# emiliofidalgo/liodom

Hardware: AMD Instinct MI355X
Metric: scans/sec (64×1800 cloud, prev_frames=20) at 1 GPU; pose RMSE vs CPU ref (higher is better)
Workload: dtype f64

## Files before the change

liodom_amd/csrc/kernels_lm.h:

```cpp
constexpr int kLmWaves = kLmThreads / 64;
__host__ __device__ __forceinline__ size_t lm_lds_bytes(int edge_cap) {
  return (size_t)((edge_cap + 3) & ~3) * sizeof(int);
}


__device__ int lm_compact_bits(const DevView& v, int s, int outer_it, int E, int* idx ) {
  const int lane = threadIdx.x & 63;
  const int Q = v.knn_queries;
  const int nb = (E + Q - 1) / Q;
  const int nwords = (nb + 3) >> 2;
  const unsigned int* mw = reinterpret_cast<const unsigned int*>(v.corr_mask + ((size_t)s * 2 + outer_it) * v.mask_stride);
  int run = 0;
  for (int w0 = 0; w0 < nwords; w0 += 64) {
    const int w = w0 + lane;
    unsigned int word = (w < nwords) ? mw[w] : 0u;
    const int pop = __popc(word);
    const int incl = wave_incl_scan_i32(pop);
    int o = run + incl - pop;
    while (word) {
      const int b = __ffs(word) - 1;
      word &= word - 1u;
      const int bit = w * 32 + b;
      idx[o++] = (bit >> 3) * Q + (bit & 7);
    }
// ... 112 lines not shown
__device__ __forceinline__ void finalize_scan(const DevView& v, int s, StreamState& st, int* sh_cnt, int eb, bool clear_hash, int ctl, int chain,
                              const double* T, int raw, bool publish_pose, const double* prev, int fc_old, int pred_copies = 3, unsigned int verdict = 1u,
                              const liodom_lm_trace_t* trace1 = nullptr) {
  __shared__ double sh_pred[19];
  const int P = v.prev_frames;
  const int tid = threadIdx.x;
  const int fc_new = fc_old + 1;
  const int nf = fc_new < P ? fc_new : P;
  const int new_slot = fc_old % P;
  int* wn = v.win_n + (size_t)s * P;
  int* wb = v.win_base + (size_t)s * (P + 1);
  int* ws = v.win_slot + (size_t)s * P;
  if (publish_pose && v.early_rebuild && tid < 50) publish_final_pose(v, s, T, raw, (unsigned int)fc_old + 1u, tid % 25, tid / 25);
  const int n_edges = st.n_edges_buf[eb];
  const int nup = st.n_used_tab[0];
  for (int j = tid; j < nf; j += blockDim.x) {
    const int sl = (fc_new - nf + j) % P;
    sh_cnt[j] = (sl == new_slot) ? n_edges : wn[sl];
    ws[j] = sl;
  }
  if (tid == 64) {
    double fin[12], q[4];
    for (int i = 0; i < 12; i++) fin[i] = T[i];
    quat_from_pose(fin, v.rotation_mode, q);
    const int k = st.scan_counter;
    st.info.scan_index = k;
    st.info.status = st.status;
    if (trace1) st.info.lm[1] = *trace1;
    if (k < v.pose_log_cap) {
      double* pl = v.pose_log + ((size_t)s * v.pose_log_cap + k) * 7;
      pl[0] = q[0]; pl[1] = q[1]; pl[2] = q[2]; pl[3] = q[3];
      pl[4] = fin[3]; pl[5] = fin[7]; pl[6] = fin[11];
      v.info_log[(size_t)s * v.pose_log_cap + k] = st.info;
    }
    st.scan_counter = k + 1;
    if (v.host_out) {
      HostOut* ho = v.host_out + (size_t)s * 2 + (k & 1);
      ho->pose[0] = q[0]; ho->pose[1] = q[1]; ho->pose[2] = q[2]; ho->pose[3] = q[3];
      ho->pose[4] = fin[3]; ho->pose[5] = fin[7]; ho->pose[6] = fin[11];
      ho->info = st.info;
      ho->pad = (int)verdict;
      __hip_atomic_store(&ho->seq, k + 1, __ATOMIC_RELEASE, __HIP_MEMORY_SCOPE_SYSTEM);
    }
    st.info.matches[0] = 0; st.info.matches[1] = 0;
  }
  if (tid == ctl) {
    double po[12];
    for (int i = 0; i < 12; i++) po[i] = prev ? prev[i] : st.prev_odom[i];
    predict_next(T, po, v.rotation_mode, sh_pred);
  }
  __syncthreads();
  if (v.pred_xch) { pred_publish(v, s, sh_pred, (unsigned int)fc_new, tid, (int)blockDim.x, pred_copies); pred_verdict_publish(v, s, (unsigned int)fc_new, verdict, tid); }
  if (tid == ctl) {
    for (int i = 0; i < 12; i++) { const double f = T[i]; st.final_odom[i] = f; st.prev_odom[i] = f; st.odom[i] = sh_pred[i]; }
    for (int i = 0; i < 4; i++) st.param_q[i] = sh_pred[12 + i];
    st.param_t[0] = sh_pred[16]; st.param_t[1] = sh_pred[17]; st.param_t[2] = sh_pred[18];
    wn[new_slot] = n_edges;
    st.frame_count = fc_new;
    st.n_frames = nf;
    int acc = 0;
    for (int j = 0; j < nf; j++) { const int c = sh_cnt[j]; sh_cnt[j] = acc; acc += c; }
    sh_cnt[nf] = acc;
    st.n_map = acc;
    if (!v.early_rebuild) st.n_used_tab[0] = 0;
    else { st.n_search = acc; st.n_filt = 0; }
    if (!chain) st.cursor = 0;
  }
  __syncthreads();
  for (int j = tid; j <= nf; j += blockDim.x) wb[j] = sh_cnt[j];
  if (clear_hash && !v.early_rebuild) hash_clear_used(v, s, nup, tid, (int)blockDim.x);
}

__device__ __forceinline__ unsigned int xcc_id() { return (unsigned int)__builtin_amdgcn_s_getreg(20 | (0 << 6) | (3 << 11)) & 0xFu; }
__device__ bool lm_exchange(const DevView& v, int s, int g, int G, unsigned int epoch,
                            double x, double* acc_total, unsigned int* status, bool local, int lane) {
  typedef __attribute__((address_space(1))) unsigned long long gu64;
  unsigned long long* base = v.lm_xch + ((size_t)s * 2 + (epoch & 1u)) * kLmGroupsMax * 64;
  INJECT_DELAY(16);
  if (lane <= 2 * kAccN) {
    unsigned long long half;
    if (lane < 2 * kAccN) {
      const unsigned long long bits = (unsigned long long)__double_as_longlong(x);
      half = (lane & 1) ? (bits >> 32) : (bits & 0xFFFFFFFFull);
    } else {
      half = xcc_id();
    }
    const unsigned long long word = ((unsigned long long)epoch << 32) | half;
    if (local) __hip_atomic_store((gu64*)(base + g * 64 + lane), word, __ATOMIC_RELAXED, __HIP_MEMORY_SCOPE_WORKGROUP);
    else __hip_atomic_store((gu64*)(base + g * 64 + lane), word, __ATOMIC_RELAXED, __HIP_MEMORY_SCOPE_AGENT);
  }
  double tot = 0.0;
  unsigned int spins = 0;
  unsigned long long t0w = 0;
  bool same = true;
  while (true) {
    bool ok = true;
    tot = 0.0;
    same = true;
    if (lane <= kAccN) {
      unsigned long long lo[kLmGroupsMax], hi[kLmGroupsMax];
      const int i0 = lane < kAccN ? 2 * lane : 2 * kAccN, i1 = lane < kAccN ? 2 * lane + 1 : 2 * kAccN;
#pragma unroll
      for (int gg = 0; gg < kLmGroupsMax; gg++) {
        const int gq = gg < G ? gg : 0;
        lo[gg] = __hip_atomic_load((gu64*)(base + gq * 64 + i0), __ATOMIC_RELAXED, __HIP_MEMORY_SCOPE_AGENT);
        hi[gg] = __hip_atomic_load((gu64*)(base + gq * 64 + i1), __ATOMIC_RELAXED, __HIP_MEMORY_SCOPE_AGENT);
      }
#pragma unroll
      for (int gg = 0; gg < kLmGroupsMax; gg++) {
        if (gg < G) {
          ok = ok && ((unsigned int)(lo[gg] >> 32) == epoch) && ((unsigned int)(hi[gg] >> 32) == epoch);
          tot += __longlong_as_double((long long)((hi[gg] << 32) | (lo[gg] & 0xFFFFFFFFull)));
          same = same && ((unsigned int)lo[gg] == (unsigned int)lo[0]);
        }
      }
    }
    if (__all(ok)) break;
    if (++spins > 4000000u || __any(wait_expired(spins, t0w))) { if (lane == 0) atomicOr(status, LIODOM_STATUS_LM_SYNC_TIMEOUT); same = false; break; }
    __builtin_amdgcn_s_sleep(1);
  }
  if (lane < kAccN) acc_total[lane] = tot;
  return __builtin_amdgcn_readlane((int)same, kAccN) != 0;
}

__device__ __forceinline__ void publish_final_pose(const DevView& v, int s, const double* T, int raw, unsigned int tag, int lane , int copy) {
  typedef __attribute__((address_space(1))) unsigned long long gu64;
  unsigned long long* base = v.pose_xch + (size_t)s * 64 + copy * 32;
  INJECT_DELAY(15);
  unsigned int word = (unsigned int)raw;
  if (lane < 24) {
    const unsigned long long bits = (unsigned long long)__double_as_longlong(T[lane >> 1]);
    word = (lane & 1) ? (unsigned int)(bits >> 32) : (unsigned int)bits;
  }
  __hip_atomic_store((gu64*)(base + lane), ((unsigned long long)tag << 32) | word, __ATOMIC_RELAXED, __HIP_MEMORY_SCOPE_AGENT);
}

__global__ void k_imu_override(DevView v, int s0, int count) {
  const int i = blockIdx.x * blockDim.x + threadIdx.x;
  if (i >= count) return;
  StreamState& st = v.state[s0 + i];
  if (!st.initialized) return;
  double odom[12], out[12], l2b[12], q[4];
#pragma unroll
  for (int k = 0; k < 12; k++) { odom[k] = st.odom[k]; l2b[k] = v.laser_to_base[k]; }
#pragma unroll
  for (int k = 0; k < 4; k++) q[k] = v.imu_q[(size_t)(s0 + i) * 4 + k];
  imu_override(odom, q, l2b, v.rotation_mode, out);
#pragma unroll
  for (int k = 0; k < 12; k++) st.odom[k] = out[k];
  quat_from_pose(out, v.rotation_mode, st.param_q);
  st.param_t[0] = out[3]; st.param_t[1] = out[7]; st.param_t[2] = out[11];
}

__device__ __forceinline__ void pose_cov_store(const DevView& v, int s, const StreamState& st, const LmState& lm, const double* acc, int nblocks, int tid) {
  const int j = tid - 64;
  if (j < 0 || j >= 21) return;
  PoseCovRaw* r = v.cov_raw + s;
  bool applied = lm.termination == LM_TERM_FUNC_TOL && lm.apply_on_ftol != 0;
  for (int k = 0; k < 4; k++) applied = applied && lm.q[k] == lm.cand_q[k];
  for (int k = 0; k < 3; k++) applied = applied && lm.t[k] == lm.cand_t[k];
  r->H[j] = applied ? acc[7 + j] : lm.H[j];
  if (j == 0) {
    r->scan_index = st.info.scan_index; r->n_res = nblocks; r->termination = lm.termination; r->has_solve = 1;
    r->cost = lm.cost;
  }
}

__device__ __forceinline__ void rebuild_beside_solve(const DevView& v, int s, StreamState& st, int eb, int outer_it, int block, int nblocks, unsigned int seq, int* sbase, int* sslot);

template <int kOuterIt, bool kChainMode>
#ifndef LIODOM_LM_WAVES_PER_SIMD
#define LIODOM_LM_WAVES_PER_SIMD 1
#endif
__global__ __launch_bounds__(kLmThreads, LIODOM_LM_WAVES_PER_SIMD) void k_lm_solve(DevView v, int s0, int eb, unsigned int seq, unsigned int done_target) {
  constexpr int outer_it = kOuterIt;
  constexpr int chain = kChainMode ? 1 : 0;
  __shared__ double sh_pose2[2][12];
  __shared__ int sh_pi, sh_ci;
  __shared__ int sh_nmoved;
  __shared__ double sh_pred_s[20];
  __shared__ int sh_unapplied;
  __shared__ double sh_acc[kAccN];
  __shared__ LmState lm;
  __shared__ int sh_flag;
  __shared__ int sh_C;
  const int s = s0 + blockIdx.y;
#if defined(LIODOM_CHAIN_PRIO)
  if (v.n_streams <= 4) __builtin_amdgcn_s_setprio(LIODOM_CHAIN_PRIO);
#endif
  const int G = v.lm_groups, gstride = G > 1 ? 8 : 1, bxl = (int)blockIdx.x;
  const bool is_solver = bxl < G * gstride && (bxl % gstride) == 0;
  const int g = is_solver ? bxl / gstride : G + (bxl < G * gstride ? bxl - (bxl / gstride + 1) : bxl - G);
  StreamState& st = v.state[s];
  __shared__ int sh_cnt[kMaxFrames + 1];
  OV_STAMP(v, bxl == 0 && threadIdx.x == 0, outer_it == 0 ? 0 : 3);
  if (seq && outer_it == 0 && bxl == 0 && threadIdx.x == 0) {
    typedef __attribute__((address_space(1))) unsigned int gu32;
    __hip_atomic_store((gu32*)(v.ov_flags + s), seq, __ATOMIC_RELAXED, __HIP_MEMORY_SCOPE_AGENT);
  }
  if (g >= G) {
    if (!v.early_rebuild || chain) return;
    __shared__ int sh_slot[kMaxFrames];
    rebuild_beside_solve(v, s, st, eb, outer_it, g - G, (int)gridDim.x - G, seq, sh_cnt, sh_slot);
    return;
  }
  __shared__ double sh_wsum[kLmWaves][32];
  __shared__ double sh_red[16][32];
  __shared__ double sh_x0[8];
  __shared__ double sh_prev[12];
  __shared__ int sh_fc;
  if (threadIdx.x < 4) sh_x0[threadIdx.x] = st.param_q[threadIdx.x];
  else if (threadIdx.x < 7) sh_x0[threadIdx.x] = st.param_t[threadIdx.x - 4];
  else if (threadIdx.x >= 64 && threadIdx.x < 76) sh_prev[threadIdx.x - 64] = st.prev_odom[threadIdx.x - 64];
  else if (threadIdx.x == 76) sh_fc = st.frame_count;
  __shared__ int sh_spec_at;
  if (threadIdx.x == 77) sh_spec_at = st.spec_eval[outer_it];
  __shared__ int sh_redo;
  if (threadIdx.x == 78) sh_redo = st.spec_redo[outer_it == 0 ? 1 : 0];
  extern __shared__ __attribute__((aligned(16))) int sh_idx[];
  const int tid = threadIdx.x;
  const bool prep = tid < kLmCtl;
  bool dead = false;
  if (chain && outer_it == 0) dead = !chain_wait_count(v.knn_done0 + s, done_target, &st.status);
  if (chain && outer_it == 0 && sh_redo) __builtin_amdgcn_fence(__ATOMIC_ACQUIRE, "agent");
  int E_in;
  if (chain && outer_it == 0) {
    typedef __attribute__((address_space(1))) unsigned int gu32;
    E_in = (int)__hip_atomic_load((gu32*)(v.edge_cnt + eb * 32 + s), __ATOMIC_RELAXED, __HIP_MEMORY_SCOPE_AGENT);
  } else {
    E_in = st.n_edges_buf[eb];
  }
  if (outer_it == 0 && tid == 0 && g == 0) {
    st.info.n_edges = E_in;
    st.info.map_points = st.n_search;
    for (int k = 0; k < 2; k++) {
      st.info.lm[k].iterations = 0; st.info.lm[k].accepted = 0; st.info.lm[k].termination = LM_TERM_NO_RESIDUALS;
      st.info.lm[k].pad = 0; st.info.lm[k].initial_cost = 0.0; st.info.lm[k].final_cost = 0.0;
    }
  }
  if (!st.initialized) {
    if (outer_it == 1 && g == 0) {
      if (seq) ov_wait_knn_done(v, s, seq, &st.status);
      if (tid == 0) st.append_raw = 1;
      __shared__ double sh_T0[12];
      if (tid < 12) sh_T0[tid] = st.odom[tid];
      __syncthreads();
      finalize_scan(v, s, st, sh_cnt, eb, true, 0, 0, sh_T0, 1, true, sh_prev, sh_fc);
      if (tid == 0) st.initialized = 1;
      if (v.cov_raw && tid == 64) {
        PoseCovRaw* r = v.cov_raw + s;
        r->scan_index = st.info.scan_index; r->n_res = 0; r->termination = st.info.lm[1].termination; r->has_solve = 0; r->cost = st.info.lm[1].final_cost;
      }
    }
    return;
  }
  bool clr_pending = outer_it == 1 && g == 0 && prep && !v.early_rebuild;
  auto clear_hash_slots = [&]() {
    hash_clear_used(v, s, st.n_used_tab[0], tid, kLmCtl);
    clr_pending = false;
  };
  const bool dbgb = (s == 0) && (g == 0) && (tid == kLmCtl) && (outer_it == 1);
  const bool dbge = (s == 0) && (g == 0) && (tid == 0) && (outer_it == 1);
  DBG_STAMP(v, dbgb, 2, 0);
  const int E = E_in;
  int nblocks = st.info.matches[outer_it];
  __shared__ int sh_nmatch;
  __shared__ double sh_scale[8];
  const unsigned int epoch0 = ((unsigned int)(st.scan_counter + 1) << 6) | ((unsigned int)outer_it << 5);
  unsigned int n_eval = 0;
  bool xch_local = false;
  LmCache cache;
  int c_lo = 0, c_hi = 0;
  int dbg_it = 0;
  auto evaluate = [&](const double* pose) {
    lm_eval(v, s, outer_it, eb, c_lo, c_hi, sh_idx, pose, &sh_wsum[0][0], cache);
    if (tid >= kLmCtl) {
      const int lane = tid - kLmCtl;
      if (G > 1) {
        const double x = lm_wave_total(&sh_wsum[0][0], c_hi - c_lo, lane >> 1);
        DBG_STAMP(v, dbgb && dbg_it < 4, 2, 12 + dbg_it);
        xch_local = lm_exchange(v, s, g, G, epoch0 | ++n_eval, x, sh_acc, &st.status, xch_local, lane);
      } else {
        if (lane < kAccN) sh_acc[lane] = lm_wave_total(&sh_wsum[0][0], c_hi - c_lo, lane);
        ++n_eval;
      }
      asm volatile("s_waitcnt lgkmcnt(0)" ::: "memory");
      __builtin_amdgcn_wave_barrier();
    }
  };
  auto my_share = [&](int C) {
    const int chunk = (C + G - 1) / G;
    c_lo = g * chunk < C ? g * chunk : C;
    c_hi = (g + 1) * chunk < C ? (g + 1) * chunk : C;
  };
  if (seq && outer_it == 1) { if (chain) dead = !chain_wait_count(v.knn_done0 + 32 + s, done_target, &st.status) || dead; else ov_wait_knn_done(v, s, seq, &st.status); }
  if (seq && outer_it == 1) { __syncthreads(); if (sh_redo) __builtin_amdgcn_fence(__ATOMIC_ACQUIRE, "agent"); }
  OV_STAMP(v, g == 0 && tid == 0 && outer_it == 1, 4);
  OV_STAMP(v, g == 0 && tid == 0 && outer_it == 0, 18);
  if (v.knn_partials) {
    const int Q = v.knn_queries;
    const int nb = (E + Q - 1) / Q;
    const double* part = v.knn_part + ((size_t)s * 2 + outer_it) * v.knn_blocks * 32;
    constexpr int kRC = kLmThreads / 32;
    const int i = tid & 31, r0 = tid >> 5;
    double x0 = 0.0, x1 = 0.0;
    if (i <= kAccN) {
      const int nb_cap = v.knn_blocks;
      for (int rb = r0; rb < (dead ? 0 : (rb == r0 ? nb_cap : nb)); rb += 16 * kRC) {
        double xs[16];
#pragma unroll
        for (int u = 0; u < 16; u++) { const int r = rb + kRC * u; xs[u] = (r < nb_cap) ? part[(size_t)r * 32 + i] : 0.0; }
#pragma unroll
        for (int u = 0; u < 16; u++) { const int r = rb + kRC * u; if (r >= nb) xs[u] = 0.0; }
#pragma unroll
        for (int u = 0; u < 16; u += 2) { x0 += xs[u]; x1 += xs[u + 1]; }
      }
    }
    sh_red[r0][i] = x0 + x1;
    __syncthreads();
    if (tid <= kAccN) {
      double x = 0.0;
#pragma unroll
      for (int r = 0; r < kRC; r++) x += sh_red[r][tid];
      if (tid < kAccN) sh_acc[tid] = x;
      else { sh_nmatch = (int)x; if (g == 0) st.info.matches[outer_it] = (int)x; }
    }
    __syncthreads();
    nblocks = sh_nmatch;
  } else {
    __syncthreads();
    if (prep) {
      const int C = lm_compact_bits(v, s, outer_it, E, sh_idx);
      if (tid == 0) sh_C = C;
    } else if (tid == kLmCtl) {
      iso_from_qt(sh_x0, sh_x0 + 4, sh_pose2[0]);
    }
    __syncthreads();
    my_share(sh_C);
    lm_cache_load(v, s, outer_it, eb, c_lo, c_hi, sh_idx, cache);
    evaluate(sh_pose2[0]);
  }
  DBG_STAMP(v, dbgb, 2, 2);
  int pi = 0, ci = -1, nmoved = 0;
  const unsigned int n_eval0 = n_eval;
  const bool spec_ok = v.speculate != 0 && v.speculate != 5 && v.speculate != 7 && g == 0 && seq != 0u && outer_it == 0;
  const bool spec_ok1 = v.speculate != 0 && v.speculate != 4 && v.speculate != 6 && g == 0 && chain != 0 && outer_it == 1 && v.early_rebuild && v.pred_xch != nullptr;
  const bool spec_forced = v.speculate == 2 || v.speculate == 6 || v.speculate == 7;
  bool spec_done = false;
  int spec_moves = -1;
  for (int step = 0;; step++) {
    if (step == 0 && tid > kLmCtl && tid <= kLmCtl + 6) {
      const int j = tid - kLmCtl - 1;
      sh_scale[j] = 1.0 / (1.0 + sqrt(sh_acc[7 + h_idx(j, j)]));
    }
    if (step == 0) __builtin_amdgcn_wave_barrier();
    if (tid == kLmCtl) {
      const int acc_before = step == 0 ? 0 : lm.accepted;
      const int f = step == 0 ? lm_begin(lm, sh_x0, sh_x0 + 4, sh_acc, nblocks, v.apply_on_ftol, sh_scale) : lm_update(lm, sh_acc);
      sh_flag = f;
      bool moved = step > 0 && lm.accepted != acc_before;
      if (step > 0 && !moved && f != LM_NEED_EVAL && lm.termination == LM_TERM_FUNC_TOL) {
        moved = true;
        for (int k = 0; k < 4; k++) moved = moved && lm.q[k] == lm.cand_q[k];
        for (int k = 0; k < 3; k++) moved = moved && lm.t[k] == lm.cand_t[k];
      }
      if (moved) { ci = pi; pi ^= 1; nmoved++; }
      if (f == LM_NEED_EVAL) iso_from_qt(lm.cand_q, lm.cand_t, sh_pose2[pi]);
      sh_pi = pi; sh_ci = ci; sh_nmoved = nmoved; sh_unapplied = (step > 0 && !moved) ? 1 : 0;
      if (step == 0) DBG_STAMP(v, dbgb, 2, 23);
    } else if (!prep) {
    } else if (step == 0 && v.knn_partials) {
      DBG_STAMP(v, dbge, 2, 24);
      const int C = dead ? 0 : lm_compact_bits(v, s, outer_it, E, sh_idx);
      if (tid == 0) sh_C = C;
      DBG_STAMP(v, dbge, 2, 25);
      my_share(C);
      lm_cache_load(v, s, outer_it, eb, c_lo, c_hi, sh_idx, cache);
    } else if (clr_pending) {
      clear_hash_slots();
    }
    __syncthreads();
    if (step == 0) { if (v.knn_partials && !prep) my_share(sh_C); DBG_STAMP(v, dbgb, 2, 3); }
    else { DBG_STAMP(v, dbgb && dbg_it < 5, 2, 5 + 2 * dbg_it); dbg_it++; }
    if (sh_flag != LM_NEED_EVAL) break;
    if ((spec_ok || spec_ok1) && !spec_done && sh_ci >= 0 &&
        (spec_forced || (!spec_forced && sh_spec_at == 0 && lm.model_cost_change <= v.spec_theta * 1e-6 * lm.cost))) {
      if (spec_ok) {
        ov_publish_pose(v, s, sh_pose2[sh_ci], &lm.q[0], seq, tid, 1);
        OV_STAMP(v, tid == 0, 19);
      } else if (tid >= kLmCtl) {
        const int l = tid - kLmCtl;
        if (l < 25) publish_final_pose(v, s, sh_pose2[sh_ci], 0, (unsigned int)sh_fc + 1u, l, 0);
        if (l == 0) predict_next(sh_pose2[sh_ci], sh_prev, v.rotation_mode, sh_pred_s);
        asm volatile("s_waitcnt lgkmcnt(0)" ::: "memory");
        __builtin_amdgcn_wave_barrier();
        pred_publish(v, s, sh_pred_s, (unsigned int)sh_fc + 1u, l, 64, 1);
        OV_STAMP(v, l == 0, 22);
      }
      if ((kInstrument && (v.debug & 64)) && tid == 0) atomicAdd(&v.dbg_clk[270], 1ull);
      spec_done = true;
      spec_moves = sh_nmoved;
    }
    const double* pose_c = sh_pose2[sh_pi];
    evaluate(pose_c);
    DBG_STAMP(v, dbgb && dbg_it < 5, 2, 4 + 2 * dbg_it);
  }
  if (clr_pending) clear_hash_slots();
  DBG_STAMP(v, dbgb, 2, 20);
  if ((kInstrument && (v.debug & 32)) && dbgb) v.dbg_clk[2 * 32 + 27] = (xch_local ? 100ull : 0ull) + 10ull * xcc_id() + (unsigned long long)n_eval;
  if (g != 0) return;
  __shared__ double sh_ov[20];
  __shared__ liodom_lm_trace_t sh_trace;
  {
    if (tid == kLmCtl) {
      sh_trace.iterations = lm.iter; sh_trace.accepted = lm.accepted; sh_trace.termination = lm.termination; sh_trace.pad = 0;
      sh_trace.initial_cost = lm.initial_cost; sh_trace.final_cost = lm.cost;
    }
    const int cif = sh_ci;
    if (cif >= 0) {
      if (tid < 12) sh_ov[tid] = sh_pose2[cif][tid];
      else if (tid >= 64 && tid < 71) sh_ov[12 + tid - 64] = (&lm.q[0])[tid - 64];
    } else if (tid == kLmCtl) {
      double q[4], t[3], T[12];
      for (int k = 0; k < 4; k++) q[k] = lm.q[k];
      for (int k = 0; k < 3; k++) t[k] = lm.t[k];
      iso_from_qt(q, t, T);
      for (int k = 0; k < 12; k++) sh_ov[k] = T[k];
      for (int k = 0; k < 4; k++) sh_ov[12 + k] = q[k];
      for (int k = 0; k < 3; k++) sh_ov[16 + k] = t[k];
    }
  }
  __syncthreads();
  if (outer_it == 0) {
    if (seq) { ov_publish_pose(v, s, sh_ov, sh_ov + 12, seq, tid, spec_done ? 2 : 3); OV_STAMP(v, tid == 0, 1); }
  } else if (v.early_rebuild && tid < 50) {
    if (tid >= 25 || !spec_done) publish_final_pose(v, s, sh_ov, 0, (unsigned int)sh_fc + 1u, tid % 25, tid / 25);
  }
  if (tid == kLmCtl) {
    if (outer_it == 0) {
      for (int k = 0; k < 4; k++) st.param_q[k] = sh_ov[12 + k];
      for (int k = 0; k < 3; k++) st.param_t[k] = sh_ov[16 + k];
      for (int k = 0; k < 12; k++) st.odom[k] = sh_ov[k];
    }
    st.spec_eval[outer_it] = (spec_done && sh_nmoved != spec_moves) ? v.spec_backoff : (sh_spec_at > 0 ? sh_spec_at - 1 : 0);
    st.spec_redo[outer_it] = (spec_done && sh_nmoved != spec_moves) ? 1 : 0;
    if (spec_done) { st.spec_stats[2 * outer_it] += 1; if (sh_nmoved != spec_moves) st.spec_stats[2 * outer_it + 1] += 1; }
    if (outer_it == 0) st.info.lm[0] = sh_trace;
    if (outer_it == 1) st.append_raw = 0;
  }
  DBG_STAMP(v, dbgb, 2, 21);
  if (outer_it == 1) {
    finalize_scan(v, s, st, sh_cnt, eb, false, kLmCtl, chain, sh_ov, 0, false, sh_prev, sh_fc, spec_done ? 2 : 3, (!spec_done || sh_nmoved == spec_moves) ? 1u : 2u, &sh_trace);
    if (v.cov_raw) pose_cov_store(v, s, st, lm, sh_acc, nblocks, tid);
    DBG_STAMP(v, dbgb, 2, 22);
  }
  DBG_STAMP(v, dbgb, 2, 28);
  OV_STAMP(v, tid == 0, outer_it == 0 ? 2 : 5);
}
```

liodom_amd/csrc/liodom_math.h:

```cpp
#pragma once
#include <cfloat>
#include <cmath>
#include <cstdint>

#if defined(__HIPCC__)
#define LD_HD __host__ __device__ __forceinline__
#define LD_UNROLL _Pragma("unroll")
#define LD_FP_CONTRACT_FAST _Pragma("clang fp contract(fast)")
#else
#define LD_HD inline
#define LD_UNROLL
#define LD_FP_CONTRACT_FAST
#endif
#if defined(__HIP_DEVICE_COMPILE__)
#define LD_RSQRT(x) rsqrt(x)
#else
#define LD_RSQRT(x) (1.0 / sqrt(x))
#endif

namespace liodom_dev {

constexpr int kJacobiSweeps = 8;
constexpr int kLmMaxIterations = 4;
constexpr double kHuberA = 0.2;
// ... 113 lines not shown
    t = 0.5 / t;
    q[0] = (T[9] - T[6]) * t;
    q[1] = (T[2] - T[8]) * t;
    q[2] = (T[4] - T[1]) * t;
  } else {
    int i = 0;
    if (T[5] > T[0]) i = 1;
    if (T[10] > (i == 0 ? T[0] : T[5])) i = 2;
    if (i == 0) quat_from_rot_case<0>(T, q);
    else if (i == 1) quat_from_rot_case<1>(T, q);
    else quat_from_rot_case<2>(T, q);
  }
}
LD_HD void iso_from_qt(const double* q, const double* t, double* T) {
  const double x = q[0], y = q[1], z = q[2], w = q[3];
  const double tx = 2 * x, ty = 2 * y, tz = 2 * z;
  const double twx = tx * w, twy = ty * w, twz = tz * w;
  const double txx = tx * x, txy = ty * x, txz = tz * x;
  const double tyy = ty * y, tyz = tz * y, tzz = tz * z;
  T[0] = 1 - (tyy + tzz); T[1] = txy - twz;       T[2] = txz + twy;        T[3] = t[0];
  T[4] = txy + twz;       T[5] = 1 - (txx + tzz); T[6] = tyz - twx;        T[7] = t[1];
  T[8] = txz - twy;       T[9] = tyz + twx;       T[10] = 1 - (txx + tyy); T[11] = t[2];
}
LD_HD void rotation_of(const double* T, int mode, double* R ) {
  double x[9] = {T[0], T[1], T[2], T[4], T[5], T[6], T[8], T[9], T[10]};
  if (mode != 0) {
    for (int it = 0; it < 24; it++) {
      double c[9];
      c[0] = x[4] * x[8] - x[5] * x[7]; c[1] = x[5] * x[6] - x[3] * x[8]; c[2] = x[3] * x[7] - x[4] * x[6];
      c[3] = x[2] * x[7] - x[1] * x[8]; c[4] = x[0] * x[8] - x[2] * x[6]; c[5] = x[1] * x[6] - x[0] * x[7];
      c[6] = x[1] * x[5] - x[2] * x[4]; c[7] = x[2] * x[3] - x[0] * x[5]; c[8] = x[0] * x[4] - x[1] * x[3];
      const double det = x[0] * c[0] + x[1] * c[1] + x[2] * c[2];
      if (!(det > 0.0) || !ld_isfinite(det)) break;
      double nx = 0.0, nc = 0.0;
      LD_UNROLL
      for (int i = 0; i < 9; i++) { nx += x[i] * x[i]; nc += c[i] * c[i]; }
      double g = 1.0;
      if (fabs(nx - 3.0) > 0.1) g = sqrt(sqrt(nc / (det * det)) / sqrt(nx));
      const double a = 0.5 * g, b = 0.5 / (g * det);
      double change = 0.0;
      LD_UNROLL
      for (int i = 0; i < 9; i++) {
        const double nv = a * x[i] + b * c[i];
        const double d = fabs(nv - x[i]);
        if (d > change) change = d;
        x[i] = nv;
      }
      if (change <= 4e-16) break;
    }
  }
  R[0] = x[0]; R[1] = x[1]; R[2] = x[2]; R[3] = T[3];
  R[4] = x[3]; R[5] = x[4]; R[6] = x[5]; R[7] = T[7];
  R[8] = x[6]; R[9] = x[7]; R[10] = x[8]; R[11] = T[11];
}
LD_HD void quat_from_pose(const double* T, int rotation_mode, double* q) {
  if (rotation_mode == 0) { quat_from_rot(T, q); return; }
  double R[12];
  rotation_of(T, rotation_mode, R);
  quat_from_rot(R, q);
}
LD_HD void transform_point(const double* T, float x, float y, float z, float* ox, float* oy,
                           float* oz) {
  const double dx = x, dy = y, dz = z;
  *ox = (float)(T[0] * dx + T[1] * dy + T[2] * dz + T[3]);
  *oy = (float)(T[4] * dx + T[5] * dy + T[6] * dz + T[7]);
  *oz = (float)(T[8] * dx + T[9] * dy + T[10] * dz + T[11]);
}
LD_HD void tf_matrix_from_quat(const double* q, double* m) {
  const double d = q[0] * q[0] + q[1] * q[1] + q[2] * q[2] + q[3] * q[3];
  const double s = 2.0 / d;
  const double xs = q[0] * s, ys = q[1] * s, zs = q[2] * s;
  const double wx = q[3] * xs, wy = q[3] * ys, wz = q[3] * zs;
  const double xx = q[0] * xs, xy = q[0] * ys, xz = q[0] * zs;
  const double yy = q[1] * ys, yz = q[1] * zs, zz = q[2] * zs;
  m[0] = 1.0 - (yy + zz); m[1] = xy - wz;         m[2] = xz + wy;
  m[3] = xy + wz;         m[4] = 1.0 - (xx + zz); m[5] = yz - wx;
  m[6] = xz - wy;         m[7] = yz + wx;         m[8] = 1.0 - (xx + yy);
}
LD_HD void tf_get_rpy(const double* m, double* roll, double* pitch, double* yaw) {
  const double kPi = 3.14159265358979323846;
  if (fabs(m[6]) >= 1) {
    *yaw = 0;
    *roll = atan2(m[7], m[8]);
    *pitch = m[6] < 0 ? kPi / 2.0 : -kPi / 2.0;
  } else {
    *pitch = -asin(m[6]);
    const double cp = cos(*pitch);
    *roll = atan2(m[7] / cp, m[8] / cp);
    *yaw = atan2(m[3] / cp, m[0] / cp);
  }
}
LD_HD void tf_set_rpy(double roll, double pitch, double yaw, double* m) {
  const double ci = cos(roll), cj = cos(pitch), ch = cos(yaw);
  const double si = sin(roll), sj = sin(pitch), sh = sin(yaw);
  const double cc = ci * ch, cs = ci * sh, sc = si * ch, ss = si * sh;
  m[0] = cj * ch; m[1] = sj * sc - cs; m[2] = sj * cc + ss;
  m[3] = cj * sh; m[4] = sj * ss + cc; m[5] = sj * cs - sc;
  m[6] = -sj;     m[7] = cj * si;      m[8] = cj * ci;
}
LD_HD void tf_quat_from_matrix(const double* m, double* q) {
  const double trace = m[0] + m[4] + m[8];
  if (trace > 0.0) {
    double s = sqrt(trace + 1.0);
    q[3] = s * 0.5;
    s = 0.5 / s;
    q[0] = (m[7] - m[5]) * s;
    q[1] = (m[2] - m[6]) * s;
    q[2] = (m[3] - m[1]) * s;
  } else {
    const int i = m[0] < m[4] ? (m[4] < m[8] ? 2 : 1) : (m[0] < m[8] ? 2 : 0);
    const int j = (i + 1) % 3, k = (i + 2) % 3;
    double s = sqrt(m[i * 3 + i] - m[j * 3 + j] - m[k * 3 + k] + 1.0);
    q[i] = s * 0.5;
    s = 0.5 / s;
    q[3] = (m[k * 3 + j] - m[j * 3 + k]) * s;
    q[j] = (m[j * 3 + i] + m[i * 3 + j]) * s;
    q[k] = (m[k * 3 + i] + m[i * 3 + k]) * s;
  }
}
LD_HD void imu_override(const double* odom, const double* imu_q, const double* laser_to_base, int rotation_mode, double* out) {
  double m[9], imu_roll, imu_pitch, imu_yaw, bl_roll, bl_pitch, bl_yaw;
  tf_matrix_from_quat(imu_q, m);
  tf_get_rpy(m, &imu_roll, &imu_pitch, &imu_yaw);
  double odom_bl[12], q_bl[4], q_new[4], l2b_inv[12];
  iso_mul(odom, laser_to_base, odom_bl);
  quat_from_pose(odom_bl, rotation_mode, q_bl);
  tf_matrix_from_quat(q_bl, m);
  tf_get_rpy(m, &bl_roll, &bl_pitch, &bl_yaw);
  tf_set_rpy(imu_roll, imu_pitch, bl_yaw, m);
  tf_quat_from_matrix(m, q_new);
  const double t_bl[3] = {odom_bl[3], odom_bl[7], odom_bl[11]};
  iso_from_qt(q_new, t_bl, odom_bl);
  iso_inverse(laser_to_base, l2b_inv);
  iso_mul(odom_bl, l2b_inv, out);
}
LD_HD void odom_message(const double* prev_odom, const double* odom, const double* laser_to_base,
                        double delta_time, int rotation_mode, double* out) {
  double bl[12], pbl[12], pinv[12], d[12], qd[4], m[9], roll, pitch, yaw;
  iso_mul(odom, laser_to_base, bl);
  quat_from_pose(bl, rotation_mode, out);
  out[4] = bl[3]; out[5] = bl[7]; out[6] = bl[11];
  iso_mul(prev_odom, laser_to_base, pbl);
  iso_inverse(pbl, pinv);
  iso_mul(pinv, bl, d);
  out[7] = d[3] / delta_time; out[8] = d[7] / delta_time; out[9] = d[11] / delta_time;
  quat_from_pose(d, rotation_mode, qd);
  tf_matrix_from_quat(qd, m);
  tf_get_rpy(m, &roll, &pitch, &yaw);
  out[10] = roll / delta_time; out[11] = pitch / delta_time; out[12] = yaw / delta_time;
}
LD_HD void quat_plus(const double* x, const double* delta, double* out) {
  LD_FP_CONTRACT_FAST
  const double u2 = delta[0] * delta[0] + delta[1] * delta[1] + delta[2] * delta[2];
  if (u2 > 0.0) {
    double s, aw;
    if (u2 < 0.25) {
      const double u = u2;
      s = 1.0 + u * (-1.0 / 6.0 + u * (1.0 / 120.0 + u * (-1.0 / 5040.0 + u * (1.0 / 362880.0 + u * (-1.0 / 39916800.0 +
          u * (1.0 / 6227020800.0 + u * (-1.0 / 1307674368000.0 + u * (1.0 / 355687428096000.0))))))));
      aw = 1.0 + u * (-0.5 + u * (1.0 / 24.0 + u * (-1.0 / 720.0 + u * (1.0 / 40320.0 + u * (-1.0 / 3628800.0 +
           u * (1.0 / 479001600.0 + u * (-1.0 / 87178291200.0 + u * (1.0 / 20922789888000.0))))))));
    } else {
      const double nd = sqrt(u2);
      s = sin(nd) / nd;
      aw = cos(nd);
    }
    const double ax = s * delta[0], ay = s * delta[1], az = s * delta[2];
    const double bw = x[3], bx = x[0], by = x[1], bz = x[2];
    out[3] = aw * bw - ax * bx - ay * by - az * bz;
    out[0] = aw * bx + ax * bw + ay * bz - az * by;
    out[1] = aw * by + ay * bw + az * bx - ax * bz;
    out[2] = aw * bz + az * bw + ax * by - ay * bx;
  } else {
    out[0] = x[0]; out[1] = x[1]; out[2] = x[2]; out[3] = x[3];
  }
}

LD_HD float sqdist_f(float qx, float qy, float qz, float mx, float my, float mz) {
  const float dx = qx - mx, dy = qy - my, dz = qz - mz;
  float r = dx * dx;
  r = r + dy * dy;
  r = r + dz * dz;
  return r;
}

LD_HD void jacobi_rot(double& app, double& aqq, double& apq, double& arp, double& arq) {
  if (fabs(apq) <= 1e-20 * (fabs(app) + fabs(aqq))) return;
  const double theta = (aqq - app) / (2.0 * apq);
  const double at = fabs(theta);
  double t = 1.0 / (at + sqrt(theta * theta + 1.0));
  if (theta < 0.0) t = -t;
  const double c = 1.0 / sqrt(t * t + 1.0);
  const double s = t * c;
  app = app - t * apq;
  aqq = aqq + t * apq;
  apq = 0.0;
  const double nrp = c * arp - s * arq;
  const double nrq = s * arp + c * arq;
  arp = nrp; arq = nrq;
}
LD_HD void eig3_sym(const double* a, double* ev) {
  double a00 = a[0], a01 = a[1], a02 = a[2], a11 = a[3], a12 = a[4], a22 = a[5];
  for (int sweep = 0; sweep < kJacobiSweeps; sweep++) {
    jacobi_rot(a00, a11, a01, a02, a12);
    jacobi_rot(a00, a22, a02, a01, a12);
    jacobi_rot(a11, a22, a12, a01, a02);
  }
  double e0 = a00, e1 = a11, e2 = a22, s;
  if (e0 > e1) { s = e0; e0 = e1; e1 = s; }
  if (e1 > e2) { s = e1; e1 = e2; e2 = s; }
  if (e0 > e1) { s = e0; e0 = e1; e1 = s; }
  ev[0] = e0; ev[1] = e1; ev[2] = e2;
}
LD_HD bool line_gate(const float* nx, const float* ny, const float* nz) {
  double cx = 0, cy = 0, cz = 0;
  for (int j = 0; j < 5; j++) { cx = cx + (double)nx[j]; cy = cy + (double)ny[j]; cz = cz + (double)nz[j]; }
  cx = cx / 5.0; cy = cy / 5.0; cz = cz / 5.0;
  double cov[6] = {0, 0, 0, 0, 0, 0};
  for (int j = 0; j < 5; j++) {
    const double zx = (double)nx[j] - cx, zy = (double)ny[j] - cy, zz = (double)nz[j] - cz;
    cov[0] = cov[0] + zx * zx; cov[1] = cov[1] + zx * zy; cov[2] = cov[2] + zx * zz;
    cov[3] = cov[3] + zy * zy; cov[4] = cov[4] + zy * zz; cov[5] = cov[5] + zz * zz;
  }
  const double p1 = cov[1] * cov[1] + cov[2] * cov[2] + cov[4] * cov[4];
  const double q = (cov[0] + cov[3] + cov[5]) / 3.0;
  const double d0 = cov[0] - q, d1 = cov[3] - q, d2 = cov[5] - q;
  const double p2 = d0 * d0 + d1 * d1 + d2 * d2 + 2.0 * p1;
  const double pp = sqrt(p2 / 6.0);
  if (pp > 0.0 && ld_isfinite(pp)) {
    const double ip = 1.0 / pp;
    const double b00 = d0 * ip, b11 = d1 * ip, b22 = d2 * ip, b01 = cov[1] * ip, b02 = cov[2] * ip, b12 = cov[4] * ip;
    double r = 0.5 * (b00 * (b11 * b22 - b12 * b12) - b01 * (b01 * b22 - b12 * b02) + b02 * (b01 * b12 - b11 * b02));
    r = r < -1.0 ? -1.0 : (r > 1.0 ? 1.0 : r);
    {
      const float s2 = (float)((1.0 - r) * (1.0 + r));
      const float phi = atan2f(sqrtf(s2 > 0.f ? s2 : 0.f), (float)r) * (1.0f / 3.0f);
      const double c_max = (double)cosf(phi), c_min = (double)cosf(phi + 2.0943951f);
      const double e_max = q + 2.0 * pp * c_max;
      const double e_min = q + 2.0 * pp * c_min;
      const double e_mid = 3.0 * q - e_max - e_min;
      const double diff = e_max - 3.0 * e_mid;
      if (fabs(diff) > 1e-4 * e_max) return diff > 0.0;
    }
    const double phi = acos(r) / 3.0;
    const double e_max = q + 2.0 * pp * cos(phi);
    const double e_min = q + 2.0 * pp * cos(phi + 2.0943951023931954923);
    const double e_mid = 3.0 * q - e_max - e_min;
    const double diff = e_max - 3.0 * e_mid;
    if (fabs(diff) > 1e-9 * e_max) return diff > 0.0;
  }
  double ev[3];
  eig3_sym(cov, ev);
  return ev[2] > 3 * ev[1];
}

constexpr int kAccN = 29;

LD_HD int h_idx(int i, int j) {
  return i * 6 - (i * (i - 1)) / 2 + (j - i);
}
LD_HD double h_at(const double* H, int i, int j) { return i <= j ? H[h_idx(i, j)] : H[h_idx(j, i)]; }

LD_HD bool residual_block(const double* Rm , const double* p, const double* a, const double* b,
                          double min_d, double max_d, double* J, double* rs, double* rho0_out, double* rho1_out) {
  LD_FP_CONTRACT_FAST
  const double tx = Rm[3], ty = Rm[7], tz = Rm[11];
  const double Rp0 = Rm[0] * p[0] + Rm[1] * p[1] + Rm[2] * p[2];
  const double Rp1 = Rm[4] * p[0] + Rm[5] * p[1] + Rm[6] * p[2];
  const double Rp2 = Rm[8] * p[0] + Rm[9] * p[1] + Rm[10] * p[2];
  const double lp0 = Rp0 + tx, lp1 = Rp1 + ty, lp2 = Rp2 + tz;
  const double u0 = lp0 - a[0], u1 = lp1 - a[1], u2 = lp2 - a[2];
  const double w0 = lp0 - b[0], w1 = lp1 - b[1], w2 = lp2 - b[2];
  const double nu0 = u1 * w2 - u2 * w1, nu1 = u2 * w0 - u0 * w2, nu2 = u0 * w1 - u1 * w0;
  const double de0 = a[0] - b[0], de1 = a[1] - b[1], de2 = a[2] - b[2];
  const double invL = LD_RSQRT(de0 * de0 + de1 * de1 + de2 * de2);
  const double cx = p[0] - tx, cy = p[1] - ty;
  const double rho_sq = cx * cx + cy * cy;
  const double inv_rho = LD_RSQRT(rho_sq);
  const double rho = rho_sq * inv_rho;
  const double inv_range = 1.0 / (max_d - min_d);
  const double w = 1.01 - (rho - min_d) * inv_range;
  const double wl = w * invL;
  const double n0 = nu0 * invL, n1 = nu1 * invL, n2 = nu2 * invL;
  const double r0 = w * n0, r1 = w * n1, r2 = w * n2;
  const double s = r0 * r0 + r1 * r1 + r2 * r2;
  const double dot = de0 * Rp0 + de1 * Rp1 + de2 * Rp2;
  const double k2 = 2.0 * wl;
  J[0]  = k2 * (Rp0 * de0 - dot); J[1]  = k2 * (Rp0 * de1);       J[2]  = k2 * (Rp0 * de2);
  J[6]  = k2 * (Rp1 * de0);       J[7]  = k2 * (Rp1 * de1 - dot); J[8]  = k2 * (Rp1 * de2);
  J[12] = k2 * (Rp2 * de0);       J[13] = k2 * (Rp2 * de1);       J[14] = k2 * (Rp2 * de2 - dot);
  const double inv_rr = inv_rho * inv_range;
  const double dwx = cx * inv_rr, dwy = cy * inv_rr;
  J[3]  = n0 * dwx;              J[4]  = wl * de2 + n0 * dwy;   J[5]  = -wl * de1;
  J[9]  = -wl * de2 + n1 * dwx;  J[10] = n1 * dwy;              J[11] = wl * de0;
  J[15] = wl * de1 + n2 * dwx;   J[16] = -wl * de0 + n2 * dwy;  J[17] = 0.0;
  double rho0, rho1;
  const double bsq = kHuberA * kHuberA;
  if (s > bsq) {
    const double inv_rr2 = LD_RSQRT(s);
    rho0 = 2.0 * kHuberA * (s * inv_rr2) - bsq;
    rho1 = kHuberA * inv_rr2;
    if (rho1 < DBL_MIN) rho1 = DBL_MIN;
  } else {
    rho0 = s; rho1 = 1.0;
  }
  double z = s * 0.0;
  LD_UNROLL
  for (int i = 0; i < 18; i++) z += J[i] * 0.0;
  *rho0_out = rho0; *rho1_out = rho1;
  rs[0] = rho1 * r0; rs[1] = rho1 * r1; rs[2] = rho1 * r2;
  return z == 0.0;
}
LD_HD double residual_entry(const double* J, const double* rs, double rho0, double rho1, int e) {
  LD_FP_CONTRACT_FAST
  if (e == 0) return 0.5 * rho0;
  if (e <= 6) { const int i = e - 1; return J[i] * rs[0] + J[6 + i] * rs[1] + J[12 + i] * rs[2]; }
  if (e >= 28) return 0.0;
  int k = e - 7, i = 0;
  while (k >= 6 - i) { k -= 6 - i; i++; }
  const int j = i + k;
  const double a0 = rho1 * J[i], a1 = rho1 * J[6 + i], a2 = rho1 * J[12 + i];
  return a0 * J[j] + a1 * J[6 + j] + a2 * J[12 + j];
}

LD_HD void residual_accumulate(const double* Rm , const double* p, const double* a,
                               const double* b, double min_d, double max_d, double* acc) {
  LD_FP_CONTRACT_FAST
  double J[18], rs[3], rho0, rho1;
// ... 424 lines not shown
```

liodom_amd/csrc/wave_ops.h:

```cpp
#pragma once
#include <hip/hip_runtime.h>

namespace liodom_dev {

constexpr int DPP_XOR1 = 0xB1;
constexpr int DPP_XOR2 = 0x4E;
constexpr int DPP_HALF_MIRROR = 0x141;
constexpr int DPP_MIRROR = 0x140;
constexpr int DPP_ROW_SHR1 = 0x111, DPP_ROW_SHR2 = 0x112, DPP_ROW_SHR4 = 0x114, DPP_ROW_SHR8 = 0x118;
constexpr int DPP_ROW_BCAST15 = 0x142, DPP_ROW_BCAST31 = 0x143;

template <int CTRL>
__device__ __forceinline__ int dpp_i32(int v) {
  return __builtin_amdgcn_update_dpp(0, v, CTRL, 0xF, 0xF, true);
}
template <int CTRL>
__device__ __forceinline__ unsigned long long dpp_u64(unsigned long long v) {
  const int lo = dpp_i32<CTRL>((int)(unsigned int)v);
  const int hi = dpp_i32<CTRL>((int)(unsigned int)(v >> 32));
  return ((unsigned long long)(unsigned int)hi << 32) | (unsigned int)lo;
}
template <int CTRL>
__device__ __forceinline__ double dpp_f64(double v) {
  return __longlong_as_double((long long)dpp_u64<CTRL>((unsigned long long)__double_as_longlong(v)));
}

__device__ __forceinline__ int xor16_i32(int v) {
  const auto r = __builtin_amdgcn_permlane16_swap((unsigned int)v, (unsigned int)v, false, false);
  const int a = (int)r[0], b = (int)r[1];
  return (a != v) ? a : b;
}
__device__ __forceinline__ int xor32_i32(int v) {
  const auto r = __builtin_amdgcn_permlane32_swap((unsigned int)v, (unsigned int)v, false, false);
  const int a = (int)r[0], b = (int)r[1];
  return (a != v) ? a : b;
}
__device__ __forceinline__ unsigned long long xor16_u64(unsigned long long v) {
  const unsigned int lo = (unsigned int)xor16_i32((int)(unsigned int)v);
  const unsigned int hi = (unsigned int)xor16_i32((int)(unsigned int)(v >> 32));
  return ((unsigned long long)hi << 32) | lo;
}
__device__ __forceinline__ unsigned long long xor32_u64(unsigned long long v) {
  const unsigned int lo = (unsigned int)xor32_i32((int)(unsigned int)v);
  const unsigned int hi = (unsigned int)xor32_i32((int)(unsigned int)(v >> 32));
  return ((unsigned long long)hi << 32) | lo;
}

__device__ __forceinline__ unsigned long long row_max_u64(unsigned long long v) {
  unsigned long long o;
  o = dpp_u64<DPP_XOR1>(v); v = o > v ? o : v;
  o = dpp_u64<DPP_XOR2>(v); v = o > v ? o : v;
  o = dpp_u64<DPP_HALF_MIRROR>(v); v = o > v ? o : v;
  o = dpp_u64<DPP_MIRROR>(v); v = o > v ? o : v;
  return v;
}
__device__ __forceinline__ unsigned long long wave_max_u64(unsigned long long v) {
  v = row_max_u64(v);
  unsigned long long o = xor16_u64(v); v = o > v ? o : v;
  o = xor32_u64(v); v = o > v ? o : v;
  return v;
}
__device__ __forceinline__ unsigned long long half_min_u64(unsigned long long v) {
  unsigned long long o;
  o = dpp_u64<DPP_XOR1>(v); v = o < v ? o : v;
  o = dpp_u64<DPP_XOR2>(v); v = o < v ? o : v;
  o = dpp_u64<DPP_HALF_MIRROR>(v); v = o < v ? o : v;
  o = dpp_u64<DPP_MIRROR>(v); v = o < v ? o : v;
  o = xor16_u64(v); v = o < v ? o : v;
  return v;
}
__device__ __forceinline__ unsigned int half_min_u32(unsigned int v) {
  unsigned int o;
  o = (unsigned int)dpp_i32<DPP_XOR1>((int)v); v = o < v ? o : v;
  o = (unsigned int)dpp_i32<DPP_XOR2>((int)v); v = o < v ? o : v;
  o = (unsigned int)dpp_i32<DPP_HALF_MIRROR>((int)v); v = o < v ? o : v;
  o = (unsigned int)dpp_i32<DPP_MIRROR>((int)v); v = o < v ? o : v;
  o = (unsigned int)xor16_i32((int)v); v = o < v ? o : v;
  return v;
}
__device__ __forceinline__ unsigned int wave_max_u32(unsigned int v) {
  unsigned int o;
  o = (unsigned int)dpp_i32<DPP_XOR1>((int)v); v = o > v ? o : v;
  o = (unsigned int)dpp_i32<DPP_XOR2>((int)v); v = o > v ? o : v;
  o = (unsigned int)dpp_i32<DPP_HALF_MIRROR>((int)v); v = o > v ? o : v;
  o = (unsigned int)dpp_i32<DPP_MIRROR>((int)v); v = o > v ? o : v;
  o = (unsigned int)xor16_i32((int)v); v = o > v ? o : v;
  o = (unsigned int)xor32_i32((int)v); v = o > v ? o : v;
  return v;
}
__device__ __forceinline__ int wave_min_i32(int v) {
  int o;
  o = dpp_i32<DPP_XOR1>(v); v = o < v ? o : v;
  o = dpp_i32<DPP_XOR2>(v); v = o < v ? o : v;
  o = dpp_i32<DPP_HALF_MIRROR>(v); v = o < v ? o : v;
  o = dpp_i32<DPP_MIRROR>(v); v = o < v ? o : v;
  o = xor16_i32(v); v = o < v ? o : v;
  o = xor32_i32(v); v = o < v ? o : v;
  return v;
}

__device__ __forceinline__ double row_sum_f64(double x) {
  x += dpp_f64<DPP_XOR1>(x);
  x += dpp_f64<DPP_XOR2>(x);
  x += dpp_f64<DPP_HALF_MIRROR>(x);
  x += dpp_f64<DPP_MIRROR>(x);
  return x;
}

__device__ __forceinline__ double fold_xor32_f64(double x, double y) {
  const unsigned long long xb = (unsigned long long)__double_as_longlong(x), yb = (unsigned long long)__double_as_longlong(y);
  const auto lo = __builtin_amdgcn_permlane32_swap((unsigned int)xb, (unsigned int)yb, false, false);
  const auto hi = __builtin_amdgcn_permlane32_swap((unsigned int)(xb >> 32), (unsigned int)(yb >> 32), false, false);
  const double a = __longlong_as_double((long long)(((unsigned long long)hi[0] << 32) | lo[0]));
  const double b = __longlong_as_double((long long)(((unsigned long long)hi[1] << 32) | lo[1]));
  return a + b;
}
__device__ __forceinline__ double fold_xor16_f64(double x, double y) {
  const unsigned long long xb = (unsigned long long)__double_as_longlong(x), yb = (unsigned long long)__double_as_longlong(y);
  const auto lo = __builtin_amdgcn_permlane16_swap((unsigned int)xb, (unsigned int)yb, false, false);
  const auto hi = __builtin_amdgcn_permlane16_swap((unsigned int)(xb >> 32), (unsigned int)(yb >> 32), false, false);
  const double a = __longlong_as_double((long long)(((unsigned long long)hi[0] << 32) | lo[0]));
  const double b = __longlong_as_double((long long)(((unsigned long long)hi[1] << 32) | lo[1]));
  return a + b;
}
template <int CTRL>
__device__ __forceinline__ double fold_dpp_f64(double x, double y, bool upper) {
  return (upper ? y : x) + dpp_f64<CTRL>(upper ? x : y);
}
__device__ __forceinline__ double wave_reduce_scatter32_f64(double (&a)[32]) {
  const int lane = (int)(threadIdx.x & 63);
#pragma unroll
  for (int j = 0; j < 16; j++) a[j] = fold_xor32_f64(a[j], a[j + 16]);
#pragma unroll
  for (int j = 0; j < 8; j++) a[j] = fold_xor16_f64(a[j], a[j + 8]);
#pragma unroll
  for (int j = 0; j < 4; j++) a[j] = fold_dpp_f64<DPP_MIRROR>(a[j], a[j + 4], (lane & 8) != 0);
#pragma unroll
  for (int j = 0; j < 2; j++) a[j] = fold_dpp_f64<DPP_HALF_MIRROR>(a[j], a[j + 2], (lane & 4) != 0);
  a[0] = fold_dpp_f64<DPP_XOR2>(a[0], a[1], (lane & 2) != 0);
  return a[0] + dpp_f64<DPP_XOR1>(a[0]);
}

__device__ __forceinline__ int wave_incl_scan_i32(int v) {
  v += __builtin_amdgcn_update_dpp(0, v, DPP_ROW_SHR1, 0xF, 0xF, true);
  v += __builtin_amdgcn_update_dpp(0, v, DPP_ROW_SHR2, 0xF, 0xF, true);
  v += __builtin_amdgcn_update_dpp(0, v, DPP_ROW_SHR4, 0xF, 0xF, true);
  v += __builtin_amdgcn_update_dpp(0, v, DPP_ROW_SHR8, 0xF, 0xF, true);
  v += __builtin_amdgcn_update_dpp(0, v, DPP_ROW_BCAST15, 0xA, 0xF, true);
  v += __builtin_amdgcn_update_dpp(0, v, DPP_ROW_BCAST31, 0xC, 0xF, true);
  return v;
}
__device__ __forceinline__ int half_incl_scan_i32(int v) {
  v += __builtin_amdgcn_update_dpp(0, v, DPP_ROW_SHR1, 0xF, 0xF, true);
  v += __builtin_amdgcn_update_dpp(0, v, DPP_ROW_SHR2, 0xF, 0xF, true);
  v += __builtin_amdgcn_update_dpp(0, v, DPP_ROW_SHR4, 0xF, 0xF, true);
  v += __builtin_amdgcn_update_dpp(0, v, DPP_ROW_SHR8, 0xF, 0xF, true);
  v += __builtin_amdgcn_update_dpp(0, v, DPP_ROW_BCAST15, 0xA, 0xF, true);
  return v;
}

__device__ __forceinline__ int readlane_i32(int v, int lane ) {
  return __builtin_amdgcn_readlane(v, lane);
}

}
```

Before: 14960.

## Run LM controller redundantly in registers across control wave instead of shared state

The LM state machine (lm_begin/lm_update) moves from a single thread operating on a shared LmState to every lane of the control wave running it redundantly on register-resident copies of the accumulators. Lane 0 writes the result back to shared memory once per step. The quaternion, translation and the speculation decision are stored beside the pose, so later consumers read them from shared memory. The change is meant to cut LDS round-trips on the serial critical path of each LM iteration. In exchange it adds register pressure from the per-lane LmState and acc copies, plus a full-struct copy to shared memory every step.

Result: slower. 14670, median of 2 (-1.9%).

```diff
diff --git a/liodom_amd/csrc/kernels_lm.h b/liodom_amd/csrc/kernels_lm.h
--- a/liodom_amd/csrc/kernels_lm.h
+++ b/liodom_amd/csrc/kernels_lm.h
@@ -288,17 +288,25 @@
   st.param_t[0] = out[3]; st.param_t[1] = out[7]; st.param_t[2] = out[11];
 }
 
-__device__ __forceinline__ void pose_cov_store(const DevView& v, int s, const StreamState& st, const LmState& lm, const double* acc, int nblocks, int tid) {
+struct LmCovOut { double H[21]; double cost; int termination; };
+__device__ __forceinline__ void pose_cov_pick(const LmState& lm, const double* acc , LmCovOut& c) {
+  bool applied = lm.termination == LM_TERM_FUNC_TOL && lm.apply_on_ftol != 0;
+#pragma unroll
+  for (int k = 0; k < 4; k++) applied = applied && lm.q[k] == lm.cand_q[k];
+#pragma unroll
+  for (int k = 0; k < 3; k++) applied = applied && lm.t[k] == lm.cand_t[k];
+#pragma unroll
+  for (int j = 0; j < 21; j++) c.H[j] = applied ? acc[7 + j] : lm.H[j];
+  c.cost = lm.cost; c.termination = lm.termination;
+}
+__device__ __forceinline__ void pose_cov_store(const DevView& v, int s, const StreamState& st, const LmCovOut& c, int nblocks, int tid) {
   const int j = tid - 64;
   if (j < 0 || j >= 21) return;
   PoseCovRaw* r = v.cov_raw + s;
-  bool applied = lm.termination == LM_TERM_FUNC_TOL && lm.apply_on_ftol != 0;
-  for (int k = 0; k < 4; k++) applied = applied && lm.q[k] == lm.cand_q[k];
-  for (int k = 0; k < 3; k++) applied = applied && lm.t[k] == lm.cand_t[k];
-  r->H[j] = applied ? acc[7 + j] : lm.H[j];
+  r->H[j] = c.H[j];
   if (j == 0) {
-    r->scan_index = st.info.scan_index; r->n_res = nblocks; r->termination = lm.termination; r->has_solve = 1;
-    r->cost = lm.cost;
+    r->scan_index = st.info.scan_index; r->n_res = nblocks; r->termination = c.termination; r->has_solve = 1;
+    r->cost = c.cost;
   }
 }
 
@@ -311,13 +319,11 @@
 __global__ __launch_bounds__(kLmThreads, LIODOM_LM_WAVES_PER_SIMD) void k_lm_solve(DevView v, int s0, int eb, unsigned int seq, unsigned int done_target) {
   constexpr int outer_it = kOuterIt;
   constexpr int chain = kChainMode ? 1 : 0;
-  __shared__ double sh_pose2[2][12];
+  __shared__ double sh_pose2[2][20];
   __shared__ int sh_pi, sh_ci;
   __shared__ int sh_nmoved;
   __shared__ double sh_pred_s[20];
-  __shared__ int sh_unapplied;
   __shared__ double sh_acc[kAccN];
-  __shared__ LmState lm;
   __shared__ int sh_flag;
   __shared__ int sh_C;
   const int s = s0 + blockIdx.y;
@@ -401,7 +407,6 @@
   const int E = E_in;
   int nblocks = st.info.matches[outer_it];
   __shared__ int sh_nmatch;
-  __shared__ double sh_scale[8];
   const unsigned int epoch0 = ((unsigned int)(st.scan_counter + 1) << 6) | ((unsigned int)outer_it << 5);
   unsigned int n_eval = 0;
   bool xch_local = false;
@@ -477,6 +482,7 @@
     evaluate(sh_pose2[0]);
   }
   DBG_STAMP(v, dbgb, 2, 2);
+  __shared__ LmState sh_lm;
   int pi = 0, ci = -1, nmoved = 0;
   const unsigned int n_eval0 = n_eval;
   const bool spec_ok = v.speculate != 0 && v.speculate != 5 && v.speculate != 7 && g == 0 && seq != 0u && outer_it == 0;
@@ -485,26 +491,52 @@
   bool spec_done = false;
   int spec_moves = -1;
   for (int step = 0;; step++) {
-    if (step == 0 && tid > kLmCtl && tid <= kLmCtl + 6) {
-      const int j = tid - kLmCtl - 1;
-      sh_scale[j] = 1.0 / (1.0 + sqrt(sh_acc[7 + h_idx(j, j)]));
-    }
-    if (step == 0) __builtin_amdgcn_wave_barrier();
-    if (tid == kLmCtl) {
+    if (!prep) {
+      const int lane = tid - kLmCtl;
+      double acc[kAccN];
+#pragma unroll
+      for (int i = 0; i < kAccN; i++) acc[i] = sh_acc[i];
+      LmState lm;
+      if (step > 0) lm = sh_lm;
       const int acc_before = step == 0 ? 0 : lm.accepted;
-      const int f = step == 0 ? lm_begin(lm, sh_x0, sh_x0 + 4, sh_acc, nblocks, v.apply_on_ftol, sh_scale) : lm_update(lm, sh_acc);
-      sh_flag = f;
+      int f;
+      if (step == 0) {
+        double sj = 0.0;
+        if (lane >= 1 && lane <= 6) sj = 1.0 / (1.0 + sqrt(sh_acc[7 + h_idx(lane - 1, lane - 1)]));
+        double scale[6];
+#pragma unroll
+        for (int j = 0; j < 6; j++) scale[j] = readlane_f64(sj, j + 1);
+        f = lm_begin(lm, sh_x0, sh_x0 + 4, acc, nblocks, v.apply_on_ftol, scale);
+      } else {
+        f = lm_update(lm, acc);
+      }
       bool moved = step > 0 && lm.accepted != acc_before;
       if (step > 0 && !moved && f != LM_NEED_EVAL && lm.termination == LM_TERM_FUNC_TOL) {
         moved = true;
+#pragma unroll
         for (int k = 0; k < 4; k++) moved = moved && lm.q[k] == lm.cand_q[k];
+#pragma unroll
         for (int k = 0; k < 3; k++) moved = moved && lm.t[k] == lm.cand_t[k];
       }
       if (moved) { ci = pi; pi ^= 1; nmoved++; }
-      if (f == LM_NEED_EVAL) iso_from_qt(lm.cand_q, lm.cand_t, sh_pose2[pi]);
-      sh_pi = pi; sh_ci = ci; sh_nmoved = nmoved; sh_unapplied = (step > 0 && !moved) ? 1 : 0;
+      const bool hand = f == LM_NEED_EVAL && (spec_ok || spec_ok1) && !spec_done && ci >= 0 &&
+                        (spec_forced || (!spec_forced && sh_spec_at == 0 && lm.model_cost_change <= v.spec_theta * 1e-6 * lm.cost));
+      if (lane == 0) {
+        if (f == LM_NEED_EVAL) {
+          double T[12];
+          iso_from_qt(lm.cand_q, lm.cand_t, T);
+#pragma unroll
+          for (int k = 0; k < 12; k++) sh_pose2[pi][k] = T[k];
+#pragma unroll
+          for (int k = 0; k < 4; k++) sh_pose2[pi][12 + k] = lm.cand_q[k];
+#pragma unroll
+          for (int k = 0; k < 3; k++) sh_pose2[pi][16 + k] = lm.cand_t[k];
+        }
+        sh_flag = f | (hand ? 2 : 0);
+        sh_pi = pi; sh_ci = ci; sh_nmoved = nmoved;
+        sh_lm = lm;
+      }
       if (step == 0) DBG_STAMP(v, dbgb, 2, 23);
-    } else if (!prep) {
     } else if (step == 0 && v.knn_partials) {
       DBG_STAMP(v, dbge, 2, 24);
       const int C = dead ? 0 : lm_compact_bits(v, s, outer_it, E, sh_idx);
@@ -518,16 +550,17 @@
     __syncthreads();
     if (step == 0) { if (v.knn_partials && !prep) my_share(sh_C); DBG_STAMP(v, dbgb, 2, 3); }
     else { DBG_STAMP(v, dbgb && dbg_it < 5, 2, 5 + 2 * dbg_it); dbg_it++; }
-    if (sh_flag != LM_NEED_EVAL) break;
-    if ((spec_ok || spec_ok1) && !spec_done && sh_ci >= 0 &&
-        (spec_forced || (!spec_forced && sh_spec_at == 0 && lm.model_cost_change <= v.spec_theta * 1e-6 * lm.cost))) {
+    const int flag = sh_flag;
+    if (!(flag & LM_NEED_EVAL)) break;
+    if (flag & 2) {
+      const double* it_pose = sh_pose2[sh_ci];
       if (spec_ok) {
-        ov_publish_pose(v, s, sh_pose2[sh_ci], &lm.q[0], seq, tid, 1);
+        ov_publish_pose(v, s, it_pose, it_pose + 12, seq, tid, 1);
         OV_STAMP(v, tid == 0, 19);
       } else if (tid >= kLmCtl) {
         const int l = tid - kLmCtl;
-        if (l < 25) publish_final_pose(v, s, sh_pose2[sh_ci], 0, (unsigned int)sh_fc + 1u, l, 0);
-        if (l == 0) predict_next(sh_pose2[sh_ci], sh_prev, v.rotation_mode, sh_pred_s);
+        if (l < 25) publish_final_pose(v, s, it_pose, 0, (unsigned int)sh_fc + 1u, l, 0);
+        if (l == 0) predict_next(it_pose, sh_prev, v.rotation_mode, sh_pred_s);
         asm volatile("s_waitcnt lgkmcnt(0)" ::: "memory");
         __builtin_amdgcn_wave_barrier();
         pred_publish(v, s, sh_pred_s, (unsigned int)sh_fc + 1u, l, 64, 1);
@@ -547,19 +580,19 @@
   if (g != 0) return;
   __shared__ double sh_ov[20];
   __shared__ liodom_lm_trace_t sh_trace;
+  __shared__ LmCovOut sh_cov;
   {
     if (tid == kLmCtl) {
-      sh_trace.iterations = lm.iter; sh_trace.accepted = lm.accepted; sh_trace.termination = lm.termination; sh_trace.pad = 0;
-      sh_trace.initial_cost = lm.initial_cost; sh_trace.final_cost = lm.cost;
+      sh_trace.iterations = sh_lm.iter; sh_trace.accepted = sh_lm.accepted; sh_trace.termination = sh_lm.termination; sh_trace.pad = 0;
+      sh_trace.initial_cost = sh_lm.initial_cost; sh_trace.final_cost = sh_lm.cost;
     }
     const int cif = sh_ci;
     if (cif >= 0) {
-      if (tid < 12) sh_ov[tid] = sh_pose2[cif][tid];
-      else if (tid >= 64 && tid < 71) sh_ov[12 + tid - 64] = (&lm.q[0])[tid - 64];
+      if (tid < 19) sh_ov[tid] = sh_pose2[cif][tid];
     } else if (tid == kLmCtl) {
       double q[4], t[3], T[12];
-      for (int k = 0; k < 4; k++) q[k] = lm.q[k];
-      for (int k = 0; k < 3; k++) t[k] = lm.t[k];
+      for (int k = 0; k < 4; k++) q[k] = sh_lm.q[k];
+      for (int k = 0; k < 3; k++) t[k] = sh_lm.t[k];
       iso_from_qt(q, t, T);
       for (int k = 0; k < 12; k++) sh_ov[k] = T[k];
       for (int k = 0; k < 4; k++) sh_ov[12 + k] = q[k];
@@ -583,11 +616,12 @@
     if (spec_done) { st.spec_stats[2 * outer_it] += 1; if (sh_nmoved != spec_moves) st.spec_stats[2 * outer_it + 1] += 1; }
     if (outer_it == 0) st.info.lm[0] = sh_trace;
     if (outer_it == 1) st.append_raw = 0;
+    if (outer_it == 1 && v.cov_raw) pose_cov_pick(sh_lm, sh_acc, sh_cov);
   }
   DBG_STAMP(v, dbgb, 2, 21);
   if (outer_it == 1) {
     finalize_scan(v, s, st, sh_cnt, eb, false, kLmCtl, chain, sh_ov, 0, false, sh_prev, sh_fc, spec_done ? 2 : 3, (!spec_done || sh_nmoved == spec_moves) ? 1u : 2u, &sh_trace);
-    if (v.cov_raw) pose_cov_store(v, s, st, lm, sh_acc, nblocks, tid);
+    if (v.cov_raw) pose_cov_store(v, s, st, sh_cov, nblocks, tid);
     DBG_STAMP(v, dbgb, 2, 22);
   }
   DBG_STAMP(v, dbgb, 2, 28);
diff --git a/liodom_amd/csrc/liodom_math.h b/liodom_amd/csrc/liodom_math.h
--- a/liodom_amd/csrc/liodom_math.h
+++ b/liodom_amd/csrc/liodom_math.h
@@ -289,6 +289,7 @@
 LD_HD void quat_plus(const double* x, const double* delta, double* out) {
   LD_FP_CONTRACT_FAST
   const double u2 = delta[0] * delta[0] + delta[1] * delta[1] + delta[2] * delta[2];
+  double o0, o1, o2, o3;
   if (u2 > 0.0) {
     double s, aw;
     if (u2 < 0.25) {
@@ -304,13 +305,14 @@
     }
     const double ax = s * delta[0], ay = s * delta[1], az = s * delta[2];
     const double bw = x[3], bx = x[0], by = x[1], bz = x[2];
-    out[3] = aw * bw - ax * bx - ay * by - az * bz;
-    out[0] = aw * bx + ax * bw + ay * bz - az * by;
-    out[1] = aw * by + ay * bw + az * bx - ax * bz;
-    out[2] = aw * bz + az * bw + ax * by - ay * bx;
+    o3 = aw * bw - ax * bx - ay * by - az * bz;
+    o0 = aw * bx + ax * bw + ay * bz - az * by;
+    o1 = aw * by + ay * bw + az * bx - ax * bz;
+    o2 = aw * bz + az * bw + ax * by - ay * bx;
   } else {
-    out[0] = x[0]; out[1] = x[1]; out[2] = x[2]; out[3] = x[3];
-  }
+    o0 = x[0]; o1 = x[1]; o2 = x[2]; o3 = x[3];
+  }
+  out[0] = o0; out[1] = o1; out[2] = o2; out[3] = o3;
 }
 
 LD_HD float sqdist_f(float qx, float qy, float qz, float mx, float my, float mz) {
diff --git a/liodom_amd/csrc/wave_ops.h b/liodom_amd/csrc/wave_ops.h
--- a/liodom_amd/csrc/wave_ops.h
+++ b/liodom_amd/csrc/wave_ops.h
@@ -163,4 +163,11 @@
   return __builtin_amdgcn_readlane(v, lane);
 }
 
+__device__ __forceinline__ double readlane_f64(double v, int lane ) {
+  const unsigned long long b = (unsigned long long)__double_as_longlong(v);
+  const unsigned int lo = (unsigned int)__builtin_amdgcn_readlane((int)(unsigned int)b, lane);
+  const unsigned int hi = (unsigned int)__builtin_amdgcn_readlane((int)(unsigned int)(b >> 32), lane);
+  return __longlong_as_double((long long)(((unsigned long long)hi << 32) | lo));
 }
+
+}
```
